# Brochu/RayTrace-WE-GPU

Hardware: AMD Instinct MI355X
Metric: Msamples/sec (pixels x spp) at 1920x1080 spp=100 depth=50 (higher is better)
Workload: dtype f32

## Files before the change

raytrace-we-gpu_amd/csrc/rtx_api.hip:

```cpp
#include <hip/hip_runtime.h>

#include <algorithm>
#include <cmath>
#include <cstdio>
#include <cstring>
#include <new>
#include <string>
#include <vector>

#include "../../include/rtx.h"
#include "rtx_internal.h"
#include "rtx_prefilter.h"

namespace {

thread_local std::string g_last_error;

int fail(int code, const std::string &msg) {
    g_last_error = msg;
    return code;
}

int hip_fail(hipError_t e, const char *what) {
    return fail(RTX_ERR_HIP, std::string(what) + ": " + hipGetErrorString(e));
// ... 724 lines not shown
    if (c->chain_n != 0 && std::memcmp(f, &c->chain_frame, sizeof *f) != 0) c->chain_n = 0;
    c->frame = *f;
    c->have_frame = true;
    return RTX_OK;
}

uint32_t rtx_part_rows(uint32_t height, uint32_t tile_rows, uint32_t part, uint32_t nparts) {
    if (tile_rows == 0 || nparts == 0 || part >= nparts) return 0;
    const uint32_t tiles = (height + tile_rows - 1) / tile_rows;
    if (part >= tiles) return 0;
    const uint32_t my_tiles = (tiles - part + nparts - 1) / nparts;
    uint32_t rows = my_tiles * tile_rows;
    const uint32_t last_tile = part + (my_tiles - 1) * nparts;
    if (last_tile == tiles - 1) rows -= tiles * tile_rows - height;
    return rows;
}

struct RefineArgs {
    const float4 *chain_in;
    float4 *chain_out;
    uint32_t samples, out_n;
    uint32_t *cost_map;
    uint32_t carry_spp;
};
static size_t chain_bytes(size_t px) { return px * (sizeof(float4) + sizeof(uint32_t)); }
static uint32_t *cost_map_of(const rtx_ctx *c) { return reinterpret_cast<uint32_t *>(c->d_chain + c->chain_pixels); }
static bool cost_map_valid(const rtx_ctx *c) { return c->d_chain && c->chain_n != 0 && c->cost_s_prev != 0; }
static int render_impl(rtx_ctx *c, uint32_t tile_rows, uint32_t part, uint32_t nparts, void *d_out,
                       float4 *accum, uint32_t accum_frames, uint32_t frame_index,
                       const RefineArgs *refine = nullptr);

static size_t sched_state_off(size_t npix) { return (2 * npix + 2 * rtx::kCostBuckets + rtx::kSchedWords + 3) & ~(size_t)3; }
constexpr uint32_t kPromCap = 65536;

int rtx_render_rows(rtx_ctx *c, uint32_t tile_rows, uint32_t part, uint32_t nparts, void *d_out) {
    if (!c) return fail(RTX_ERR_INVALID, "rtx_render_rows: null ctx");
    return render_impl(c, tile_rows, part, nparts, d_out, nullptr, 0, c->frame.frame_index);
}

int rtx_accumulate(rtx_ctx *c, int reset) {
    if (!c) return fail(RTX_ERR_INVALID, "rtx_accumulate: null ctx");
    if (!c->have_frame) return fail(RTX_ERR_STATE, "rtx_accumulate: no frame set");
    int rc = set_device(c);
    if (rc) return rc;
    const size_t px = (size_t)c->frame.width * c->frame.height;
    if (reset || c->accum_frames == 0 || !c->d_accum || c->accum_pixels != px) {
        if (!c->d_accum || c->accum_pixels != px) {
            RTX_HIP(hipStreamSynchronize(c->stream));
            (void)hipFree(c->d_accum);
            c->d_accum = nullptr;
            c->accum_pixels = 0;
            RTX_HIP(hipMalloc(&c->d_accum, px * sizeof(float4)));
            c->accum_pixels = px;
        }
        RTX_HIP(hipMemsetAsync(c->d_accum, 0, px * sizeof(float4), c->stream));
        c->accum_frames = 0;
    }
    rc = render_impl(c, 1, 0, 1, nullptr, c->d_accum, c->accum_frames + 1, c->accum_frames);
    if (rc == RTX_OK) c->accum_frames++;
    return rc;
}

uint32_t rtx_accumulated_frames(rtx_ctx *c) { return c ? c->accum_frames : 0; }

int rtx_render_sum(rtx_ctx *c, uint32_t frame_index, void *d_sum) {
    if (!c) return fail(RTX_ERR_INVALID, "rtx_render_sum: null ctx");
// ... 99 lines not shown
        p.chain_in = refine->chain_in;
        p.chain_out = refine->chain_out;
        p.out_n = refine->out_n;
    }

    if (c->ev_count == c->events.size()) {
        EventPair &old = c->events[c->ev_head];
        const hipError_t q = hipEventQuery(old.stop);
        if (q == hipSuccess) {
            float t = 0.0f;
            RTX_HIP(hipEventElapsedTime(&t, old.start, old.stop));
            c->ms_folded += t;
            c->ev_head = (c->ev_head + 1) % c->events.size();
            c->ev_count--;
        } else if (q == hipErrorNotReady) {
            std::vector<EventPair> grown(2 * c->events.size());
            for (size_t i = 0; i < c->ev_count; ++i) grown[i] = c->events[(c->ev_head + i) % c->events.size()];
            c->events.swap(grown);
            c->ev_head = 0;
        } else {
            return hip_fail(q, "hipEventQuery");
        }
    }
    EventPair &ev = c->events[(c->ev_head + c->ev_count) % c->events.size()];
    if (!ev.start) RTX_HIP(hipEventCreate(&ev.start));
    if (!ev.stop) RTX_HIP(hipEventCreate(&ev.stop));
    RTX_HIP(hipEventRecord(ev.start, c->stream));
    const size_t npix = (size_t)rows * f.width;
    if (c->sched_pixels < npix) {
        RTX_HIP(hipStreamSynchronize(c->stream));
        (void)hipFree(c->d_sched);
        c->d_sched = nullptr;
        c->sched_pixels = 0;
        RTX_HIP(hipMalloc(&c->d_sched,
                          (sched_state_off(npix) + 4 * npix + 8 * (size_t)kPromCap + 5 * npix) * sizeof(uint32_t)));
        RTX_HIP(hipMemsetAsync(c->d_sched + sched_state_off(npix) + 4 * npix, 0,
                               8 * (size_t)kPromCap * sizeof(uint32_t), c->stream));
        c->sched_pixels = npix;
    }
    const size_t ps_need = rtx::ps_scratch_floats(p);
    if (ps_need > c->ps_floats) {
        RTX_HIP(hipStreamSynchronize(c->stream));
        (void)hipFree(c->d_ps);
        c->d_ps = nullptr;
        c->ps_floats = 0;
        RTX_HIP(hipMalloc(&c->d_ps, ps_need * sizeof(float)));
        c->ps_floats = ps_need;
    }
    rtx::KSchedule sched;
    sched.ps_scratch = c->d_ps;
    sched.ps_floats = c->ps_floats;
    sched.cost = c->d_sched;
    sched.perm = c->d_sched + c->sched_pixels;
    sched.buckets = c->d_sched + 2 * c->sched_pixels;
    sched.state = reinterpret_cast<float4 *>(c->d_sched + sched_state_off(c->sched_pixels));
    sched.npix = (uint32_t)c->sched_pixels;
    sched.nbuckets = rtx::kCostBuckets;
    sched.tune = c->tune;
    if (!c->aux_stream) {
        RTX_HIP(hipStreamCreateWithFlags(&c->aux_stream, hipStreamNonBlocking));
        RTX_HIP(hipEventCreateWithFlags(&c->ev_fork, hipEventDisableTiming));
        RTX_HIP(hipEventCreateWithFlags(&c->ev_join, hipEventDisableTiming));
    }
    sched.aux = c->aux_stream;
    sched.prom_q = c->d_sched + sched_state_off(c->sched_pixels) + 4 * c->sched_pixels;
    sched.prom_cap = kPromCap;
    sched.stage = reinterpret_cast<float4 *>(sched.prom_q + 8 * (size_t)kPromCap);
    sched.inv = sched.prom_q + 8 * (size_t)kPromCap + 4 * c->sched_pixels;
    sched.epoch = (uint32_t)++c->epoch;
    sched.ev_fork = c->ev_fork;
    sched.ev_join = c->ev_join;
    sched.cost_map = refine ? refine->cost_map : nullptr;
    sched.carry_spp = refine ? refine->carry_spp : 0u;
    hipError_t e = rtx::launch_render(p, sched, c->stream);
    if (e != hipSuccess) return hip_fail(e, "launch_render");
    RTX_HIP(hipEventRecord(ev.stop, c->stream));
    c->ev_count++;
    c->launches++;
    c->samples += (uint64_t)rows * f.width * p.spp;
    return RTX_OK;
}

int rtx_render(rtx_ctx *c) { return rtx_render_rows(c, 1, 0, 1, nullptr); }

int rtx_refine(rtx_ctx *c, uint32_t samples, int reset) {
    if (!c) return fail(RTX_ERR_INVALID, "rtx_refine: null ctx");
    if (samples == 0) return fail(RTX_ERR_INVALID, "rtx_refine: samples is 0");
    if (!c->have_world) return fail(RTX_ERR_STATE, "rtx_refine: no world uploaded");
    if (!c->have_frame) return fail(RTX_ERR_STATE, "rtx_refine: no frame set");
    if (c->frame.rng_mode == RTX_RNG_PER_SAMPLE)
        return fail(RTX_ERR_INVALID, "rtx_refine: the per-sample RNG has no chain to continue (rtx_accumulate is its "
                                     "progressive form)");
    const size_t px = (size_t)c->frame.width * c->frame.height;
    const bool fresh = reset || c->chain_n == 0 || !c->d_chain || c->chain_pixels != px ||
                       std::memcmp(&c->frame, &c->chain_frame, sizeof c->frame) != 0;
    const uint32_t have = fresh ? 0u : c->chain_n;
    if (samples > 0xffffffffu - have) return fail(RTX_ERR_INVALID, "rtx_refine: more than 2^32 - 1 samples in all");
    int rc = set_device(c);
    if (rc) return rc;
    if (!c->d_chain || c->chain_pixels != px) {
        RTX_HIP(hipStreamSynchronize(c->stream));
// ... 373 lines not shown
```

raytrace-we-gpu_amd/csrc/rtx_diag.h:

```cpp
#pragma once

#include "rtx_internal.h"

#ifndef RTX_DIAG_PROF
#define RTX_DIAG_PROF 0
#endif
#ifndef RTX_DIAG_PIXEL
#define RTX_DIAG_PIXEL 0
#endif
#ifndef RTX_DIAG_COOP
#define RTX_DIAG_COOP 0
#endif
#ifndef RTX_DIAG_RAYS
#define RTX_DIAG_RAYS 0
#endif

namespace rtx {
namespace {

#if RTX_DIAG_PROF
__device__ __forceinline__ uint32_t *diag_slots() {
    __shared__ uint32_t s[4][8];
    return s[(threadIdx.x / 64) & 3u];
}
__device__ __forceinline__ void diag_add(int k, uint32_t v) {
    const uint64_t m = __ballot(1);
    if ((int)(threadIdx.x & 63u) == __ffsll((long long)m) - 1) diag_slots()[k] += v;
}
#define RTX_DIAG_ADD(k, v) diag_add(k, v)
__device__ __forceinline__ unsigned long long *diag_hw() {
    __shared__ unsigned long long s[4][8];
    return s[(threadIdx.x / 64) & 3u];
}
__device__ __forceinline__ void diag_hw_clock(int k) {
    const uint64_t m = __ballot(1);
    if ((int)(threadIdx.x & 63u) == __ffsll((long long)m) - 1) {
        const unsigned long long tn = __builtin_readcyclecounter();
        if (k >= 0) diag_hw()[k] += tn - diag_hw()[3];
        diag_hw()[3] = tn;
    }
}
__device__ __forceinline__ void diag_hw_walk(uint32_t steps, uint32_t rounds) {
    uint32_t mx = 0;
    for (int b = 7; b >= 0; --b) {
        const uint32_t t = mx | (1u << b);
        if (__ballot(min(steps, 255u) >= t) != 0ull) mx = t;
    }
    const uint64_t m = __ballot(1);
    if ((int)(threadIdx.x & 63u) == __ffsll((long long)m) - 1) {
        diag_hw()[4] += 1ull;
        diag_hw()[5] += mx;
        diag_hw()[7] += rounds ? rounds : mx;
    }
    atomicAdd(&diag_hw()[6], (unsigned long long)steps);
}
#define RTX_DIAG_HW_BEGIN() diag_hw_clock(-1)
#define RTX_DIAG_HW(k) diag_hw_clock(k)
#define RTX_DIAG_WALK(steps, rounds) diag_hw_walk(steps, rounds)
#else
#define RTX_DIAG_ADD(k, v)
#define RTX_DIAG_HW_BEGIN()
#define RTX_DIAG_HW(k)
#define RTX_DIAG_WALK(steps, rounds)
#endif

#define RTX_CP(k)                                                   \
    if (RTX_DIAG_COOP && cp) {                                      \
        const unsigned long long tn = __builtin_readcyclecounter(); \
        cp[k] += tn - *tq;                                          \
        *tq = tn;                                                   \
    }

struct Diag {
#if RTX_DIAG_RAYS
    uint32_t rit = 0;
#endif
#if RTX_DIAG_PROF
    unsigned long long pr[7] = {0, 0, 0, 0, 0, 0, 0};
    unsigned long long tq = 0;
#endif
#if RTX_DIAG_COOP
    unsigned long long cpa[8] = {0, 0, 0, 0, 0, 0, 0, 0};
    unsigned long long ctq = 0;
    bool was_coop = false;
#endif
    __device__ __forceinline__ void begin() {
#if RTX_DIAG_PROF
        if ((threadIdx.x & 63u) == 0u)
            for (int k = 0; k < 8; ++k) diag_slots()[k] = 0u, diag_hw()[k] = 0ull;
        tq = __builtin_readcyclecounter();
#endif
#if RTX_DIAG_COOP
        ctq = __builtin_readcyclecounter();
#endif
    }
    __device__ __forceinline__ void section(int k) {
#if RTX_DIAG_PROF
        const unsigned long long tn = __builtin_readcyclecounter();
        pr[k] += tn - tq;
        tq = tn;
#else
        (void)k;
#endif
    }
    __device__ __forceinline__ void iteration(uint64_t act) {
#if RTX_DIAG_PROF
        pr[4]++;
        pr[6] += __popcll(act);
#else
        (void)act;
#endif
    }
    __device__ __forceinline__ void tail_iteration() {
#if RTX_DIAG_PROF
        pr[5]++;
#endif
    }
    __device__ __forceinline__ unsigned long long *coop_begin(uint32_t tier, unsigned long long *&tqp) {
#if RTX_DIAG_COOP
        tqp = &ctq;
        if (tier != (uint32_t)RTX_DIAG_COOP) return nullptr;
        const unsigned long long tn = __builtin_readcyclecounter();
// ... 15 lines not shown
        }
        was_coop = tier == (uint32_t)RTX_DIAG_COOP;
#else
        (void)cp;
        (void)tier;
#endif
    }
    __device__ __forceinline__ void rays(const KParams &P, f3 o, f3 d, bool live, uint32_t slot) {
#if RTX_DIAG_RAYS
        if (!P.wave_times) return;
        const uint32_t w = blockIdx.x * (blockDim.x / 64u) + threadIdx.x / 64u;
        if ((++rit + w * 13u) % (uint32_t)RTX_DIAG_RAYS != 0u) return;
        unsigned long long r = 0;
        if ((threadIdx.x & 63u) == 0u) r = atomicAdd(&P.wave_times[0], 1ull);
        r = __shfl(r, 0, 64);
        const unsigned long long base = 64ull + 256ull * r;
        if (base + 256ull > 2ull * P.wave_cap) return;
        auto pk = [](float a, float b) {
            return ((unsigned long long)__float_as_uint(b) << 32) | __float_as_uint(a);
        };
        unsigned long long *q = P.wave_times + base + 4u * (threadIdx.x & 63u);
        q[0] = pk(o.x, o.y);
        q[1] = pk(o.z, d.x);
        q[2] = pk(d.y, d.z);
        q[3] = ((unsigned long long)slot << 32) | (live ? 1u : 0u);
#else
        (void)P, (void)o, (void)d, (void)live, (void)slot;
#endif
    }
    __device__ __forceinline__ void finish(const KParams &P) {
#if RTX_DIAG_PROF
        if (P.wave_times && (threadIdx.x & 63u) == 0u) {
            for (int k = 0; k < 7; ++k) atomicAdd(&P.wave_times[k], pr[k]);
            for (int k = 0; k < 7; ++k) atomicAdd(&P.wave_times[8 + k], (unsigned long long)diag_slots()[k]);
            if (P.wave_cap >= 12u)
                for (int k = 0; k < 8; ++k) atomicAdd(&P.wave_times[16 + k], diag_hw()[k]);
        }
#endif
#if RTX_DIAG_COOP
        if (P.wave_times && (threadIdx.x & 63u) == 0u)
            for (int k = 0; k < 6; ++k) atomicAdd(&P.wave_times[k], cpa[k]);
#endif
        (void)P;
    }
};

__device__ __forceinline__ void diag_pixel_start(const KParams &P, uint32_t gid, unsigned long long mode) {
#if RTX_DIAG_PIXEL
    if (P.wave_times && gid < P.wave_cap) P.wave_times[2 * gid] = (__builtin_amdgcn_s_memrealtime() << 2) | mode;
#else
    (void)P;
    (void)gid;
    (void)mode;
#endif
}
__device__ __forceinline__ void diag_pixel_end(const KParams &P, uint32_t gid) {
#if RTX_DIAG_PIXEL
    if (P.wave_times && gid < P.wave_cap) P.wave_times[2 * gid + 1] = __builtin_amdgcn_s_memrealtime();
#else
    (void)P;
    (void)gid;
#endif
}
constexpr bool kDiagAny = RTX_DIAG_PROF || RTX_DIAG_PIXEL || RTX_DIAG_COOP || RTX_DIAG_RAYS;

}
}
```

raytrace-we-gpu_amd/csrc/rtx_internal.h:

```cpp
#pragma once

#include <hip/hip_runtime.h>
#include <stdint.h>

#include "rtx_grid.h"
#include "rtx_refine_keys.h"

struct rtx_ctx;

namespace rtx {

struct KScene {
    const float *soa;
    const float *pre;
    const float4 *pre4;
    const float4 *cen;
    const int *mtype;
    const float4 *mval;
    uint32_t n, n_pad;
    float smag;
    float flat_cy;
    uint32_t flat_lo, flat_hi;
    const float *cpre;
    const float *cbnd;
// ... 62 lines not shown
    float4 *accum;
    uint32_t accum_frames;
    unsigned long long *wave_times;
    uint32_t wave_cap;
    const uint32_t *perm;
    uint32_t *cost_out;
    uint32_t cost_spp;
    uint32_t cost_cap;
    uint32_t cost_capped;
    uint32_t *pre_done;
    uint32_t pre_stop;
    float4 *state;
    uint32_t prio_slots;
    uint32_t coop_max;
    uint32_t prio_t1, prio_t2, prio_hot;
    uint32_t trace_ext;
    uint32_t chunk;
    uint32_t *prom;
    uint32_t *errors;
    unsigned long long *err_diag;
    uint32_t *prom_q;
    uint32_t prom_cap, prom_min, epoch;
    uint32_t *heavy;
    const uint32_t *cost_in;
    float dyn_bar[3];
    uint32_t trace_lg;
    float *ps_scratch;
    uint32_t ps_px, ps_cap;
    const float4 *chain_in;
    float4 *chain_out;
    uint32_t out_n;
    uint32_t *cost_map;
    uint32_t carry_spp;
};

struct KTune {
    double a1, a1_small, a1_low, a2_small, a2_medium, a2_large, rho, rho_low, rho2, prio_frac;
    double occ_small, occ_low, occ_normal;
    uint32_t coop_max;
    uint32_t coop_max_large;
    uint32_t prio_t1, prio_t2, prio_hot;
    uint32_t chunk;
    double trace_small, trace_low, trace_medium, trace_large;
    double prom_small, prom_low, prom_medium, prom_large;
    double prom_big;
    uint32_t trace_group;
    double trace_solo;
    uint32_t cap_split;
    double dyn1, dyn2, dyn3;
};
KTune default_tune();

struct KSchedule {
    uint32_t *cost;
    uint32_t *perm;
    float4 *state;
    float4 *stage;
    uint32_t *inv;
    uint32_t *buckets;
    uint32_t npix;
    uint32_t nbuckets;
    float *ps_scratch;
    size_t ps_floats;
    KTune tune;
    hipStream_t aux;
    hipEvent_t ev_fork, ev_join;
    uint32_t *prom_q;
    uint32_t prom_cap;
    uint32_t epoch;
    uint32_t *cost_map;
    uint32_t carry_spp;
};
constexpr uint32_t kSchedWords = 16;
constexpr uint32_t kBlock = 256;

hipError_t launch_render(const KParams &p, const KSchedule &sched, hipStream_t stream);
size_t ps_scratch_floats(const KParams &p);
hipError_t launch_cost(const KParams &p, hipStream_t stream);
hipError_t launch_deinterleave(const float4 *gathered, float4 *image, uint32_t width,
                               uint32_t height, uint32_t tile_rows, uint32_t nparts,
                               uint32_t max_rows, hipStream_t stream);
hipError_t launch_fold_frames(float4 *accum, const float4 *sums, uint32_t m, size_t slot_pixels, size_t pixels,
                              uint32_t divisor, float4 *image, hipStream_t stream);
hipError_t launch_chain_image(const float4 *chain, float4 *image, size_t pixels, uint32_t n, hipStream_t stream);
hipError_t launch_debug_hit_world(const KScene &s, const float *rays, uint32_t nrays,
                                  float t_min, float t_max, uint32_t start_block, float *out,
                                  hipStream_t stream);
bool debug_scan_rate_supported(const KParams &p);
hipError_t launch_debug_scan_rate(const KParams &p, uint32_t reps, unsigned long long *sink, uint32_t *waves,
                                  hipStream_t stream);
hipError_t launch_debug_math(int fn, const float *in0, const float *in1, uint32_t n,
// ... 8 lines not shown
```

raytrace-we-gpu_amd/csrc/rtx_kernels.hip:

```cpp
#include <algorithm>
#include <cstdlib>
#include <cstring>
#include <mutex>
#include <type_traits>
#include <vector>

#include "rtx_device_math.h"
#include "rtx_diag.h"
#include "rtx_internal.h"
#include "rtx_prefilter.h"

#if defined(__HIP_DEVICE_COMPILE__) && !defined(__gfx950__)
#error "rtx_kernels.hip targets gfx950 (MI355X) only"
#endif

namespace rtx {

namespace {

constexpr float kTMin = 0.001f;

struct FrameVals {
    f3 org, hor, ver, llc;
    float img_w, img_h;
// ... 1472 lines not shown
    return true;
}

template <bool kCost = false, bool kRefine = false>
__device__ __forceinline__ bool shade(const KParams &P, const Frame &F, Lane &L, int hit, float t,
                                      uint32_t prom_thr = 0u) {
    L.segs++;
    f3 c;
    const int r = path_segment(P, L, hit, t, c);
    if (r == kSegSky) L.acc = L.acc + c;
    const bool ended = r != kSegContinue;
    if (ended) {
        L.sample++;
        if (L.sample >= P.spp) {
            write_pixel<kCost, kRefine>(P, L);
            L.active = false;
            diag_pixel_end(P, L.gid);
        } else if (!kCost && prom_thr != 0u && promote<kRefine>(P, L, prom_thr)) {
            L.active = false;
            return true;
        } else {
            begin_sample(P, F, L.x, L.y, L);
        }
    } else if (kCost && P.cost_cap != 0u && L.segs - L.seg0 >= P.cost_cap) {
        P.cost_out[L.gid] = P.cost_capped;
        P.state[L.gid] = make_float4(0.0f, 0.0f, 0.0f, __uint_as_float(0x7fc00000u));
        L.segs = L.seg0;
        L.active = false;
        diag_pixel_end(P, L.gid);
    }
    return false;
}

__device__ __forceinline__ void lane_pixel(const KParams &P, uint32_t gid, uint32_t &x, uint32_t &y) {
    const uint32_t lr = gid / P.width;
    x = gid - lr * P.width;
    const uint32_t j = lr / P.tile_rows;
    const uint32_t w = lr - j * P.tile_rows;
    y = (j * P.nparts + P.part) * P.tile_rows + w;
}

__device__ __forceinline__ void count_segments(const KParams &P, uint32_t segs) {
#pragma unroll
    for (int off = 32; off > 0; off >>= 1) segs += __shfl_xor(segs, off, 64);
    if ((threadIdx.x & 63u) == 0u && segs != 0u) atomicAdd(P.counters, (unsigned long long)segs);
}

#ifndef RTX_CHECK_KERNARG
#define RTX_CHECK_KERNARG 0
#endif
__device__ __forceinline__ Frame load_frame(const KParams &P) {
    if constexpr (RTX_CHECK_KERNARG != 0) {
        const FrameVals v = frame_vals();
        const bool same = __float_as_uint(v.img_w) == __float_as_uint(P.img_w) &&
                          __float_as_uint(v.img_h) == __float_as_uint(P.img_h) &&
                          __float_as_uint(v.org.x) == __float_as_uint(P.org[0]) &&
                          __float_as_uint(v.llc.z) == __float_as_uint(P.llc[2]) &&
                          __float_as_uint(v.lens_r) == __float_as_uint(P.lens_r);
        if (!same && P.errors && (threadIdx.x & 63u) == 0u) atomicOr(P.errors, kErrKernarg);
    }
    return Frame{};
}

template <bool kRefine = false>
__device__ __forceinline__ void start_pixel(const KParams &P, const Frame &F, uint32_t gid, Lane &L) {
    L.gid = gid;
    lane_pixel(P, gid, L.x, L.y);
    L.seg0 = L.segs;
    const float4 st = P.state && !P.cost_out ? P.state[gid] : make_float4(0.f, 0.f, 0.f, 0.f);
    L.c0 = 0u;
    if (P.state && !P.cost_out && !__builtin_isnan(st.w)) {
        L.acc = mk3(st.x, st.y, st.z);
        L.sample = P.cost_spp;
        L.seed = st.w;
        if constexpr (kRefine) {
            L.c0 = P.cost_map[gid];
        } else if (P.cost_in) {
            L.c0 = P.cost_in[gid];
        }
    } else {
        L.acc = mk3(0.0f, 0.0f, 0.0f);
        L.sample = 0;
        L.seed = pixel_seed(P, L.x, L.y, 0);
        if constexpr (kRefine) {
            if (P.chain_in) {
                const float4 ch = P.chain_in[gid];
                L.acc = mk3(ch.x, ch.y, ch.z);
                L.seed = ch.w;
            }
            if (P.carry_spp != 0u) L.c0 = P.cost_map[gid];
        }
        if (P.state && !P.cost_out) L.seg0 |= kSeg0Restart;
    }
    L.active = true;
    begin_sample(P, F, L.x, L.y, L);
}

__device__ __forceinline__ void set_prio(uint32_t p) {
    switch (__builtin_amdgcn_readfirstlane(p)) {
        case 0: __builtin_amdgcn_s_setprio(0); break;
        case 1: __builtin_amdgcn_s_setprio(1); break;
        case 2: __builtin_amdgcn_s_setprio(2); break;
        default: __builtin_amdgcn_s_setprio(3); break;
    }
}

template <bool kRefine = false>
__device__ __forceinline__ uint32_t dyn_level(const KParams &P, const Lane &L, float m) {
    float rem = 0.0f;
    if (L.active) {
        const bool rs = (L.seg0 & kSeg0Restart) != 0u;
        const float segs = (float)(L.segs - (L.seg0 & ~kSeg0Restart) + L.c0);
        rem = rs && L.sample == 0u ? 3.0e38f : segs * (float)(P.spp - L.sample) / (float)max(L.sample, 1u);
        if constexpr (kRefine) {
            const float all = (float)(L.segs - (L.seg0 & ~kSeg0Restart)) + (float)L.c0;
            rem = rs && L.sample == 0u ? 3.0e38f
                                       : all * (float)(P.spp - L.sample) /
                                             fmaxf((float)L.sample + (float)P.carry_spp, 1.0f);
        }
    }
    return __ballot(rem > P.dyn_bar[2] * m) != 0ull   ? 3u
           : __ballot(rem > P.dyn_bar[1] * m) != 0ull ? 2u
           : __ballot(rem > P.dyn_bar[0] * m) != 0ull ? 1u
                                                      : 0u;
}

template <bool kRefine = false>
__device__ __forceinline__ bool refill(const KParams &P, const Frame &F, uint32_t lo, uint32_t hi, Lane &L) {
    const uint64_t idle = __ballot(!L.active);
    if (idle == 0ull) return false;
    const uint32_t cnt = (uint32_t)__popcll(idle);
    if (P.chunk > 1u) {
        const uint32_t lane = threadIdx.x & 63u;
        const uint32_t rank = (uint32_t)__popcll(idle & ((1ull << lane) - 1ull));
        const uint32_t avail = L.ce - L.cb;
        uint32_t nb = 0, n = 0;
        if (cnt > avail) {
            n = cnt - avail;
            if (L.cb < hi - (hi - lo) / 8u) n = max(n, P.chunk);
            if (lane == 0u) nb = atomicAdd(P.queue, n);
            nb = lo + (uint32_t)__shfl((int)nb, 0, 64);
        }
        if (!L.active) {
            const uint32_t g = rank < avail ? L.cb + rank : nb + (rank - avail);
            if (g < hi) {
                start_pixel<kRefine>(P, F, P.perm ? P.perm[g] : g, L);
                L.slot = g;
                diag_pixel_start(P, L.gid, 0);
            }
        }
        if (cnt > avail) {
            L.cb = nb + (cnt - avail);
            L.ce = min(nb + n, hi);
            return L.cb >= hi;
        }
        L.cb += cnt;
        return false;
    }
    const int leader = __ffsll((long long)idle) - 1;
    const uint32_t lane = threadIdx.x & 63u;
    uint32_t base = 0;
    if ((int)lane == leader) base = atomicAdd(P.queue, cnt);
    base = lo + __shfl(base, leader, 64);
    if (!L.active) {
        const uint32_t g = base + (uint32_t)__popcll(idle & ((1ull << lane) - 1ull));
        if (g < hi) {
            start_pixel<kRefine>(P, F, P.perm ? P.perm[g] : g, L);
            L.slot = g;
            diag_pixel_start(P, L.gid, 0);
        }
    }
    return base + cnt >= hi;
}

struct HeavyState {
    uint32_t k1, kh;
    bool t1_done, t2_done;
    uint32_t tier;
};
template <bool kRefine = false>
__device__ __forceinline__ bool take_from(const KParams &P, const Frame &F, uint32_t *ctr, uint32_t lo, uint32_t hi,
                                          uint32_t room, uint64_t act, Lane &L, bool &done) {
    const uint32_t lane = threadIdx.x & 63u;
    uint32_t h = 0;
    if (lane == 0u) h = atomicAdd(ctr, room);
    h = lo + __shfl(h, 0, 64);
    if (h >= hi) {
        done = true;
        return false;
    }
    const uint32_t take = min(room, hi - h);
    const uint32_t rk = (uint32_t)__popcll(~act & ((1ull << lane) - 1ull));
    if (!L.active && rk < take) {
        start_pixel<kRefine>(P, F, P.perm[h + rk], L);
        L.slot = h + rk;
        diag_pixel_start(P, L.gid, ctr == P.heavy ? 1ull : 2ull);
    }
    if (h + room >= hi) done = true;
    return true;
}
template <bool kRefine = false>
__device__ __forceinline__ void take_heavy(const KParams &P, const Frame &F, HeavyState &H, Lane &L) {
    const uint64_t act = __ballot(L.active);
    const uint32_t have = (uint32_t)__popcll(act);
    if (have == 0u) H.tier = 0;
    if (have == 0u && !H.t1_done && take_from<kRefine>(P, F, P.heavy, 0, H.k1, kHeavy1, act, L, H.t1_done)) {
        H.tier = 1;
        return;
    }
    if (H.tier == 1u) return;
    if (!H.t2_done && have < kHeavy2 && take_from<kRefine>(P, F, P.heavy + 2, H.k1, H.kh, kHeavy2 - have, act, L, H.t2_done))
        H.tier = 2;
}

template <uint32_t kLg, typename Src>
__device__ __forceinline__ void trace_group_segment(const KParams &P, const Frame &F, const Src &src, Lane &W,
                                                    bool &ended) {
    constexpr uint32_t lg = kLg;
    const KScene &S = P.scene;
    const uint32_t lane = threadIdx.x & 63u;
    const uint32_t g = 1u << lg, k = lane & (g - 1u);
    const uint64_t gm = lg >= 6u ? ~0ull : ((1ull << g) - 1ull) << (lane & ~(g - 1u));
    const float inf = __uint_as_float(0x7f800000u);
    const int last = (int)S.n - 1;
    const ScatterSpec sp = scatter_spec(W.seed);
    LineTest T = line_test_setup(W.o.x, W.o.y, W.o.z, W.d.x, W.d.y, W.d.z, W.a, S.smag);
    if (lg < 6u && !W.active) {
        T.ux = T.uy = T.uz = T.vy = T.vz = T.nou = T.nov = 0.0f;
        T.thr = inf;
    }
    const f2v ux = {T.ux, T.ux}, uy = {T.uy, T.uy}, uz = {T.uz, T.uz}, vy = {T.vy, T.vy}, vz = {T.vz, T.vz};
    const f2v nou = {T.nou, T.nou}, nov = {T.nov, T.nov}, th = {T.thr, T.thr};
    uint64_t key = hit_key(inf, -1);
    bool ok = true;
    const uint32_t nsteps = src.npairs >> lg;
#pragma unroll 1
    for (uint32_t s0 = 0; s0 < nsteps; s0 += kGfSteps) {
        uint32_t im = 0;
        const uint32_t s1 = min(s0 + kGfSteps, nsteps);
        auto step = [&](uint32_t st) {
            f2v cx, cy, cz, R;
            src.pair((st << lg) + k, cx, cy, cz, R);
            const f2v pu = fma2(cx, ux, fma2(cy, uy, fma2(cz, uz, nou)));
            const f2v pv = fma2(cy, vy, fma2(cz, vz, nov));
// ... 264 lines not shown
    if (kPF && threadIdx.x == 0) *pack = 0u;
    if (prom_on && threadIdx.x == 0) s_server = 0u;
    if (prom_on && blockIdx.x == 0 && threadIdx.x == 0)
        __hip_atomic_store(&P.prom[3], 1u, __ATOMIC_RELAXED, __HIP_MEMORY_SCOPE_AGENT);
    if (coop_lds || kPF || prom_on) __syncthreads();
    const int last = (int)P.scene.n - 1;
    const Frame F = load_frame(P);
    const uint32_t npix = P.rows_local * P.width;
    const unsigned long long t_start = P.wave_times ? __builtin_amdgcn_s_memrealtime() : 0ull;
    Lane L;
    L.active = false;
    L.segs = 0;
    L.slot = ~0u;
    L.cb = L.ce = 0u;
    bool exhausted = !kPersist;
    if (!kPersist) {
        const uint32_t gid = tile_pixel(blockIdx.x * kRB + threadIdx.x, P.width, P.rows_local, kExactTile);
        if (gid < npix) start_pixel<kRefine>(P, F, gid, L);
    }
    HeavyState H;
    H.kh = (kPersist && P.heavy) ? min(P.heavy[1], npix) : 0u;
    H.k1 = (kPersist && P.heavy) ? min(P.heavy[3], H.kh) : 0u;
    H.t1_done = H.k1 == 0u || P.trace_ext != 0u;
    H.t2_done = H.k1 == H.kh;
    H.tier = 0;
    const uint32_t kh = H.kh;
    const float dyn_m = (kPersist && P.cost_in && P.heavy) ? __uint_as_float(P.heavy[5]) : 0.0f;
    const uint32_t owned = npix - (P.trace_ext != 0u ? H.k1 : 0u);
    uint32_t written = 0;
    unsigned long long last_beat = 0;
    Diag D;
    D.begin();
    for (;;) {
        if (!(H.t1_done && H.t2_done) && (H.tier != 0u || __ballot(L.active) == 0ull)) take_heavy<kRefine>(P, F, H, L);
        if (H.tier != 0u && __ballot(L.active) == 0ull) H.tier = 0;
        const bool heavy = H.tier != 0u;
        if (!heavy && !exhausted) exhausted = refill<kRefine>(P, F, kh, npix, L);
        if (kPersist && kCost && P.pre_done && exhausted && pre_stop(P, npix, L)) continue;
        const uint64_t act = __ballot(L.active);
        D.section(0);
        if (act == 0ull) {
            if (!prom_on) break;
            if (written != 0u && (threadIdx.x & 63u) == 0u)
                __hip_atomic_fetch_add(&P.prom[2], written, __ATOMIC_RELAXED, __HIP_MEMORY_SCOPE_AGENT);
            written = 0;
            uint32_t srv = 0;
            if ((threadIdx.x & 63u) == 0u) srv = atomicCAS(&s_server, 0u, threadIdx.x / 64u + 1u);
            srv = (uint32_t)__builtin_amdgcn_readfirstlane(__shfl((int)srv, 0, 64));
            if (srv != 0u && srv != threadIdx.x / 64u + 1u) break;
            if (!take_promoted<kRefine>(P, F, npix, owned, false, L)) {
                if ((threadIdx.x & 63u) == 0u) atomicExch(&s_server, 0u);
                break;
            }
            L.active = (threadIdx.x & 63u) == 0u;
            H.tier = 1;
            continue;
        }
        const uint64_t was_active = act;
        if (prom_on) beat(P, last_beat);
        D.iteration(act);
        if (heavy || (exhausted && (uint32_t)__popcll(act) <= P.coop_max)) {
            D.tail_iteration();
            float my_best = __uint_as_float(0x7f800000u);
            bool my_seq = false;
            set_prio(H.tier == 1u ? P.prio_t1 : H.tier == 2u ? P.prio_t2 : (uint32_t)kTailPrio);
            unsigned long long *ctqp;
            unsigned long long *cp = D.coop_begin(H.tier, ctqp);
            bool promoted = false;
            int my_hit = kCulled
                             ? hit_world_groups_culled(P.scene, act, L.active, L.o, L.d, L.a, L.inv_a, kTMin, coop_ws,
// ... 159 lines not shown
    const uint32_t k1 = min(P.heavy[3], min(P.heavy[1], npix));
    const uint32_t k0 = min(P.heavy[4], k1);
    const uint32_t lane = threadIdx.x & 63u;
    const uint32_t lg_many = min(max(P.trace_lg, 3u), 6u);
    set_prio(P.prio_t1);
    uint32_t lg = 6u;
    Lane W;
    W.active = false;
    W.segs = 0;
    W.seg0 = 0;
    W.slot = 0;
    uint32_t segs = 0;
    bool t1_done = k1 == 0u;
    bool serve_done = P.prom == nullptr;
    unsigned long long last_beat = 0;
    for (;;) {
        uint64_t act = __ballot(W.active);
        if (act == 0ull && t1_done) lg = lg_many;
        if (!t1_done) {
            if (act == 0ull) {
                const uint32_t next = (uint32_t)__builtin_amdgcn_readfirstlane(
                    __hip_atomic_load(P.heavy, __ATOMIC_RELAXED, __HIP_MEMORY_SCOPE_AGENT));
                lg = next < k0 ? 6u : lg_many;
            }
            const uint32_t g = 1u << lg;
            const uint64_t need = __ballot(!W.active && (lane & (g - 1u)) == 0u);
            if (need != 0ull) {
                const uint32_t n = (uint32_t)__popcll(need);
                uint32_t base = 0;
                if (lane == 0u) base = atomicAdd(P.heavy, n);
                base = (uint32_t)__builtin_amdgcn_readfirstlane(__shfl((int)base, 0, 64));
                const uint32_t rank = (uint32_t)__popcll(need & ((1ull << (lane & ~(g - 1u))) - 1ull));
                if (!W.active && base + rank < k1) {
                    start_pixel<kRefine>(P, F, P.perm[base + rank], W);
                    W.slot = base + rank;
                    diag_pixel_start(P, W.gid, 1ull);
                }
                if (base + n >= k1) t1_done = true;
                act = __ballot(W.active);
            }
        }
        if (t1_done && !serve_done) {
            const uint32_t g = 1u << lg;
            const uint64_t need = __ballot(!W.active && (lane & (g - 1u)) == 0u);
            if (need != 0ull) {
                set_prio(P.prio_t1);
                if (take_promoted_groups<kRefine>(P, F, npix, npix - k1, need, lg, act == 0ull, W) < 0) serve_done = true;
                set_prio(P.prio_t1);
                act = __ballot(W.active);
            }
        }
        if (act == 0ull) {
            if (t1_done && serve_done) break;
            continue;
        }
        if (t1_done && lg < 6u) {
            uint32_t m = 0;
            for (uint32_t r = 0; r < (64u >> lg); ++r) m += (uint32_t)((act >> (r << lg)) & 1ull);
            if (2u * m <= (64u >> lg)) {
                const uint32_t nlg = 6u - (m <= 1u ? 0u : 32u - (uint32_t)__builtin_clz(m - 1u));
                regroup(W, lg, nlg, act);
                lg = nlg;
            }
        }
        bool ended;
        const bool first = (lane & ((1u << lg) - 1u)) == 0u;
        if (lg == 6u) {
            uint32_t n = 0;
// ... 53 lines not shown
constexpr uint32_t kChunkShare = 16;

__global__ void __launch_bounds__(kBlock) k_cost_hist(const uint32_t *cost, uint32_t width, uint32_t rows,
                                                      uint32_t cost_spp, uint32_t sat_cap, uint32_t tile,
                                                      uint32_t tile_y, uint32_t *counts) {
    __shared__ uint32_t h[kCostBuckets];
    for (uint32_t b = threadIdx.x; b < kCostBuckets; b += kBlock) h[b] = 0;
    __syncthreads();
    const uint32_t base = blockIdx.x * kBlock * kSortPerThread;
    for (uint32_t k = 0; k < kSortPerThread; ++k) {
        const uint32_t i = tile_pixel(base + k * kBlock + threadIdx.x, width, rows, tile, tile_y);
        if (i != ~0u) atomicAdd(&h[cost_key(cost, i, width, rows, cost_spp, sat_cap)], 1u);
    }
    __syncthreads();
    for (uint32_t b = threadIdx.x; b < kCostBuckets; b += kBlock)
        if (h[b]) atomicAdd(&counts[b], h[b]);
}
__global__ void __launch_bounds__(kBlock) k_carried_hist(const uint32_t *map, uint32_t width, uint32_t rows,
                                                         uint32_t s_prev, uint32_t tile, uint32_t tile_y,
                                                         uint32_t *counts) {
    __shared__ uint32_t h[kCostBuckets];
    for (uint32_t b = threadIdx.x; b < kCostBuckets; b += kBlock) h[b] = 0;
    __syncthreads();
    const uint32_t base = blockIdx.x * kBlock * kSortPerThread;
    for (uint32_t k = 0; k < kSortPerThread; ++k) {
        const uint32_t i = tile_pixel(base + k * kBlock + threadIdx.x, width, rows, tile, tile_y);
        if (i != ~0u) atomicAdd(&h[carried_key(map, i, width, rows, s_prev)], 1u);
    }
    __syncthreads();
    for (uint32_t b = threadIdx.x; b < kCostBuckets; b += kBlock)
        if (h[b]) atomicAdd(&counts[b], h[b]);
}

__global__ void __launch_bounds__(kBlock) k_cost_scatter(const uint32_t *cost, uint32_t width, uint32_t rows,
                                                         uint32_t cost_spp, uint32_t sat_cap, uint32_t tile,
                                                         uint32_t tile_y,
                                                         const uint32_t *counts, uint32_t *cursors,
                                                         uint32_t *perm, uint32_t *inv) {
    __shared__ uint32_t h[kCostBuckets], start[kCostBuckets];
    for (uint32_t b = threadIdx.x; b < kCostBuckets; b += kBlock) h[b] = 0;
    __syncthreads();
    const uint32_t base = blockIdx.x * kBlock * kSortPerThread;
    uint32_t rank[kSortPerThread], key[kSortPerThread];
    for (uint32_t k = 0; k < kSortPerThread; ++k) {
        const uint32_t i = tile_pixel(base + k * kBlock + threadIdx.x, width, rows, tile, tile_y);
        key[k] = i != ~0u ? cost_key(cost, i, width, rows, cost_spp, sat_cap) : 0u;
        rank[k] = i != ~0u ? atomicAdd(&h[key[k]], 1u) : 0u;
    }
    __syncthreads();
    if (threadIdx.x == 0) {
        uint32_t pre = 0;
        for (uint32_t b = 0; b < kCostBuckets; ++b) {
            start[b] = pre;
            pre += counts[b];
        }
    }
    __syncthreads();
    for (uint32_t b = threadIdx.x; b < kCostBuckets; b += kBlock)
        if (h[b]) start[b] += atomicAdd(&cursors[b], h[b]);
    __syncthreads();
    for (uint32_t k = 0; k < kSortPerThread; ++k) {
        const uint32_t i = tile_pixel(base + k * kBlock + threadIdx.x, width, rows, tile, tile_y);
        if (i != ~0u) {
            const uint32_t g = start[key[k]] + rank[k];
            perm[g] = i;
            if (inv) inv[i] = g;
        }
    }
}
__global__ void __launch_bounds__(kBlock) k_carried_scatter(const uint32_t *map, uint32_t width, uint32_t rows,
                                                            uint32_t s_prev, uint32_t tile, uint32_t tile_y,
                                                            const uint32_t *counts, uint32_t *cursors,
                                                            uint32_t *perm, uint32_t *inv) {
    __shared__ uint32_t h[kCostBuckets], start[kCostBuckets];
    for (uint32_t b = threadIdx.x; b < kCostBuckets; b += kBlock) h[b] = 0;
    __syncthreads();
    const uint32_t base = blockIdx.x * kBlock * kSortPerThread;
    uint32_t rank[kSortPerThread], key[kSortPerThread];
    for (uint32_t k = 0; k < kSortPerThread; ++k) {
        const uint32_t i = tile_pixel(base + k * kBlock + threadIdx.x, width, rows, tile, tile_y);
        key[k] = i != ~0u ? carried_key(map, i, width, rows, s_prev) : 0u;
        rank[k] = i != ~0u ? atomicAdd(&h[key[k]], 1u) : 0u;
    }
    __syncthreads();
    if (threadIdx.x == 0) {
        uint32_t pre = 0;
        for (uint32_t b = 0; b < kCostBuckets; ++b) {
            start[b] = pre;
            pre += counts[b];
        }
    }
    __syncthreads();
    for (uint32_t b = threadIdx.x; b < kCostBuckets; b += kBlock)
        if (h[b]) start[b] += atomicAdd(&cursors[b], h[b]);
    __syncthreads();
    for (uint32_t k = 0; k < kSortPerThread; ++k) {
        const uint32_t i = tile_pixel(base + k * kBlock + threadIdx.x, width, rows, tile, tile_y);
        if (i != ~0u) {
            const uint32_t g = start[key[k]] + rank[k];
            perm[g] = i;
            if (inv) inv[i] = g;
        }
    }
}

}
KTune default_tune() {
    KTune t;
    t.a1 = kHeavy1Alpha;
    t.a1_small = kHeavy1AlphaSmall;
    t.a1_low = kHeavy1AlphaLow;
    t.a2_small = kHeavyAlpha;
    t.a2_medium = kHeavy2AlphaMedium;
    t.a2_large = kHeavy2AlphaLarge;
    t.rho = kHeavyRho;
    t.rho_low = kHeavyRhoLow;
    t.rho2 = kHeavyRho2;
    t.prio_frac = kPrioFracX100 / 100.0;
    t.occ_small = t.occ_low = t.occ_normal = 1.0;
    t.coop_max = (uint32_t)kCoopMax;
    t.coop_max_large = (uint32_t)kCoopMaxLarge;
    t.prio_t1 = 3;
    t.prio_t2 = 2;
    t.prio_hot = 3;
    t.chunk = 64;
    t.trace_small = kTraceSmall;
    t.trace_low = kTraceLow;
    t.trace_medium = kTraceMedium;
    t.trace_large = kTraceLarge;
    t.prom_small = kPromSmall;
    t.prom_low = kPromLow;
    t.prom_medium = kPromMedium;
    t.prom_large = kPromLarge;
    t.prom_big = kPromBig;
// ... 615 lines not shown
            c.pre_stop = (uint32_t)(kPreStopFrac * (double)pblocks * kRB);
        }
        launch_kr<true, true>(p.scene, pblocks, lds, stream, c);
    } else {
        launch_kr<false, true>(p.scene, need_x, lds, stream, c);
    }
#ifndef RTX_QUEUE_TILE_ALL
#define RTX_QUEUE_TILE_ALL 0
#endif
#ifndef RTX_QUEUE_TILE_SPLIT
#define RTX_QUEUE_TILE_SPLIT 0
#endif
    uint32_t qtile = RTX_QUEUE_TILE_ALL || (double)lanes >= tune.rho * (double)min(need, resident_blocks(render_fn<true, false>(p.scene), lds)) * kRB
                         ? kQueueTile
                         : 0u;
    uint32_t qtile_y = 0u;
    if (RTX_QUEUE_TILE_SPLIT != 0 && p.nparts > 1u && p.tile_rows != 0u) qtile = RTX_QUEUE_TILE_SPLIT, qtile_y = p.tile_rows;
    const uint32_t sblocks = ceil_div(tile_span(p.width, p.rows_local, qtile, qtile_y), kBlock * kSortPerThread);
    if (carried)
        hipLaunchKernelGGL(k_carried_hist, dim3(sblocks), dim3(kBlock), 0, stream, sched.cost_map, p.width,
                           p.rows_local, sched.carry_spp, qtile, qtile_y, sched.buckets);
    else
        hipLaunchKernelGGL(k_cost_hist, dim3(sblocks), dim3(kBlock), 0, stream, sched.cost, p.width,
                           p.rows_local, c.spp, split_cap, qtile, qtile_y, sched.buckets);
    uint32_t blocks = min(need, resident_blocks(render_fn<true, false>(p.scene), lds));
    {
        const double px_per_lane = (double)lanes / ((double)blocks * kRB);
        const double occ = px_per_lane < tune.rho ? tune.occ_small : px_per_lane < tune.rho_low ? tune.occ_low : tune.occ_normal;
        blocks = max(1u, (uint32_t)(blocks * occ + 0.5));
    }
    uint32_t *heavy = sched.buckets + 2 * kCostBuckets;
    hipLaunchKernelGGL(k_heavy_split, dim3(1), dim3(64), 0, stream, sched.buckets, (uint32_t)lanes, blocks * kRB, p.spp,
                       heavy, tune);
    if (carried)
        hipLaunchKernelGGL(k_carried_scatter, dim3(sblocks), dim3(kBlock), 0, stream, sched.cost_map, p.width,
                           p.rows_local, sched.carry_spp, qtile, qtile_y, sched.buckets, sched.buckets + kCostBuckets,
                           sched.perm, sched.stage ? sched.inv : nullptr);
    else
        hipLaunchKernelGGL(k_cost_scatter, dim3(sblocks), dim3(kBlock), 0, stream, sched.cost, p.width,
                           p.rows_local, c.spp, split_cap, qtile, qtile_y, sched.buckets, sched.buckets + kCostBuckets, sched.perm,
                           sched.stage ? sched.inv : nullptr);
    KParams q = p;
    q.cost_spp = carried ? 0u : c.spp;
    q.perm = sched.perm;
    q.out_slot = sched.stage;
    q.stage_tag = sched.epoch;
    q.state = carried ? nullptr : sched.state;
    q.carry_spp = carried ? sched.carry_spp : 0u;
    q.prio_slots = (uint32_t)((double)blocks * kRB * tune.prio_frac);
    q.heavy = heavy;
    if (tune.dyn1 > 0.0) {
        q.cost_in = carried ? sched.cost_map : sched.cost;
        q.dyn_bar[0] = (float)tune.dyn1;
        q.dyn_bar[1] = (float)tune.dyn2;
        q.dyn_bar[2] = (float)tune.dyn3;
    }
    {
        const double ppl = (double)lanes / ((double)blocks * kRB);
        q.chunk = (!pf && ppl >= tune.rho2) ? min(tune.chunk, 4096u)
                  : ppl >= tune.rho_low     ? min(tune.chunk, kChunkShare)
                                            : 0u;
    }
    e = hipMemsetAsync(p.queue, 0, sizeof(uint32_t), stream);
    if (e != hipSuccess) return e;
    uint32_t trace_waves = 0;
    if (sched.aux && !pf && p.scene.n <= kCoopLds) {
        const double px_per_lane = (double)lanes / ((double)blocks * kRB);
        const double frac = px_per_lane < tune.rho ? tune.trace_small : px_per_lane < tune.rho_low ? tune.trace_low
                            : px_per_lane < tune.rho2 ? tune.trace_medium : tune.trace_large;
        trace_waves = (uint32_t)(frac * blocks * (kRB / 64) + 0.5);
    }
    {
        const double px_per_lane = (double)lanes / ((double)blocks * kRB);
        const double pm = p.scene.n > kCoopLds    ? tune.prom_big
                          : px_per_lane < tune.rho ? tune.prom_small : px_per_lane < tune.rho_low ? tune.prom_low
                          : px_per_lane < tune.rho2 ? tune.prom_medium : tune.prom_large;
        if (pm > 0.0 && sched.prom_q && sched.prom_cap > 0) {
// ... 105 lines not shown
```

Baseline: 6477.

## Precompute packed per-slot start records in scatter kernel to cut dependent loads

The cost/carried scatter kernels now also write a 32-byte start record per sorted slot, holding pixel index, coordinates, c0 cost and resume state. The render kernel's refill and heavy-take paths then load one contiguous record instead of chasing perm[g] and then gathering state[gid], cost_in[gid] and recomputing pixel coordinates. This is meant to replace a dependent chain of scattered loads at pixel start with coalesced sequential loads. In exchange it adds extra global writes in the scatter pass and 8 words per pixel of scratch memory. Optional diagnostic counters for load latency are added as well.

Result: no change. 6516, median of 6 (+0.6%).

```diff
diff --git a/raytrace-we-gpu_amd/csrc/rtx_api.hip b/raytrace-we-gpu_amd/csrc/rtx_api.hip
--- a/raytrace-we-gpu_amd/csrc/rtx_api.hip
+++ b/raytrace-we-gpu_amd/csrc/rtx_api.hip
@@ -780,6 +780,9 @@
 
 static size_t sched_state_off(size_t npix) { return (2 * npix + 2 * rtx::kCostBuckets + rtx::kSchedWords + 3) & ~(size_t)3; }
 constexpr uint32_t kPromCap = 65536;
+static size_t sched_rec_off(size_t npix) {
+    return (sched_state_off(npix) + 4 * npix + 8 * (size_t)kPromCap + 5 * npix + 7) & ~(size_t)7;
+}
 
 int rtx_render_rows(rtx_ctx *c, uint32_t tile_rows, uint32_t part, uint32_t nparts, void *d_out) {
     if (!c) return fail(RTX_ERR_INVALID, "rtx_render_rows: null ctx");
@@ -945,8 +948,7 @@
         (void)hipFree(c->d_sched);
         c->d_sched = nullptr;
         c->sched_pixels = 0;
-        RTX_HIP(hipMalloc(&c->d_sched,
-                          (sched_state_off(npix) + 4 * npix + 8 * (size_t)kPromCap + 5 * npix) * sizeof(uint32_t)));
+        RTX_HIP(hipMalloc(&c->d_sched, (sched_rec_off(npix) + 8 * npix) * sizeof(uint32_t)));
         RTX_HIP(hipMemsetAsync(c->d_sched + sched_state_off(npix) + 4 * npix, 0,
                                8 * (size_t)kPromCap * sizeof(uint32_t), c->stream));
         c->sched_pixels = npix;
@@ -980,6 +982,7 @@
     sched.prom_cap = kPromCap;
     sched.stage = reinterpret_cast<float4 *>(sched.prom_q + 8 * (size_t)kPromCap);
     sched.inv = sched.prom_q + 8 * (size_t)kPromCap + 4 * c->sched_pixels;
+    sched.rec = reinterpret_cast<uint4 *>(c->d_sched + sched_rec_off(c->sched_pixels));
     sched.epoch = (uint32_t)++c->epoch;
     sched.ev_fork = c->ev_fork;
     sched.ev_join = c->ev_join;
diff --git a/raytrace-we-gpu_amd/csrc/rtx_diag.h b/raytrace-we-gpu_amd/csrc/rtx_diag.h
--- a/raytrace-we-gpu_amd/csrc/rtx_diag.h
+++ b/raytrace-we-gpu_amd/csrc/rtx_diag.h
@@ -20,7 +20,7 @@
 
 #if RTX_DIAG_PROF
 __device__ __forceinline__ uint32_t *diag_slots() {
-    __shared__ uint32_t s[4][8];
+    __shared__ uint32_t s[4][16];
     return s[(threadIdx.x / 64) & 3u];
 }
 __device__ __forceinline__ void diag_add(int k, uint32_t v) {
@@ -28,6 +28,16 @@
     if ((int)(threadIdx.x & 63u) == __ffsll((long long)m) - 1) diag_slots()[k] += v;
 }
 #define RTX_DIAG_ADD(k, v) diag_add(k, v)
+#if RTX_DIAG_PROF >= 2
+__device__ __forceinline__ unsigned long long diag_loads_begin() { return __builtin_readcyclecounter(); }
+__device__ __forceinline__ void diag_loads_end(unsigned long long t0) {
+    asm volatile("s_waitcnt vmcnt(0)" ::: "memory");
+    diag_add(7, (uint32_t)(__builtin_readcyclecounter() - t0));
+}
+#define RTX_DIAG_LOADS_BEGIN() const unsigned long long diag_ld0 = diag_loads_begin()
+#define RTX_DIAG_LOADS_END() diag_loads_end(diag_ld0)
+#define RTX_DIAG_START_END() (diag_add(8, (uint32_t)(__builtin_readcyclecounter() - diag_ld0)), diag_add(9, 1u))
+#endif
 __device__ __forceinline__ unsigned long long *diag_hw() {
     __shared__ unsigned long long s[4][8];
     return s[(threadIdx.x / 64) & 3u];
@@ -63,6 +73,11 @@
 #define RTX_DIAG_HW(k)
 #define RTX_DIAG_WALK(steps, rounds)
 #endif
+#ifndef RTX_DIAG_LOADS_BEGIN
+#define RTX_DIAG_LOADS_BEGIN() ((void)0)
+#define RTX_DIAG_LOADS_END() ((void)0)
+#define RTX_DIAG_START_END() ((void)0)
+#endif
 
 #define RTX_CP(k)                                                   \
     if (RTX_DIAG_COOP && cp) {                                      \
@@ -87,7 +102,7 @@
     __device__ __forceinline__ void begin() {
 #if RTX_DIAG_PROF
         if ((threadIdx.x & 63u) == 0u)
-            for (int k = 0; k < 8; ++k) diag_slots()[k] = 0u, diag_hw()[k] = 0ull;
+            for (int k = 0; k < 8; ++k) diag_slots()[k] = diag_slots()[8 + k] = 0u, diag_hw()[k] = 0ull;
         tq = __builtin_readcyclecounter();
 #endif
 #if RTX_DIAG_COOP
@@ -169,9 +184,11 @@
 #if RTX_DIAG_PROF
         if (P.wave_times && (threadIdx.x & 63u) == 0u) {
             for (int k = 0; k < 7; ++k) atomicAdd(&P.wave_times[k], pr[k]);
-            for (int k = 0; k < 7; ++k) atomicAdd(&P.wave_times[8 + k], (unsigned long long)diag_slots()[k]);
+            for (int k = 0; k < 8; ++k) atomicAdd(&P.wave_times[8 + k], (unsigned long long)diag_slots()[k]);
             if (P.wave_cap >= 12u)
                 for (int k = 0; k < 8; ++k) atomicAdd(&P.wave_times[16 + k], diag_hw()[k]);
+            if (P.wave_cap >= 16u)
+                for (int k = 0; k < 8; ++k) atomicAdd(&P.wave_times[24 + k], (unsigned long long)diag_slots()[8 + k]);
         }
 #endif
 #if RTX_DIAG_COOP
diff --git a/raytrace-we-gpu_amd/csrc/rtx_internal.h b/raytrace-we-gpu_amd/csrc/rtx_internal.h
--- a/raytrace-we-gpu_amd/csrc/rtx_internal.h
+++ b/raytrace-we-gpu_amd/csrc/rtx_internal.h
@@ -118,6 +118,18 @@
     uint32_t out_n;
     uint32_t *cost_map;
     uint32_t carry_spp;
+    const uint4 *rec;
+};
+
+constexpr uint32_t kRecResume = 0u;
+constexpr uint32_t kRecRestart = 1u;
+constexpr uint32_t kRecFresh = 2u;
+constexpr uint32_t kRecKindShift = 30u;
+struct KRecArgs {
+    uint4 *rec;
+    const float4 *state;
+    const uint32_t *c0;
+    uint32_t tile_rows, part, nparts;
 };
 
 struct KTune {
@@ -143,6 +155,7 @@
     float4 *state;
     float4 *stage;
     uint32_t *inv;
+    uint4 *rec;
     uint32_t *buckets;
     uint32_t npix;
     uint32_t nbuckets;
diff --git a/raytrace-we-gpu_amd/csrc/rtx_kernels.hip b/raytrace-we-gpu_amd/csrc/rtx_kernels.hip
--- a/raytrace-we-gpu_amd/csrc/rtx_kernels.hip
+++ b/raytrace-we-gpu_amd/csrc/rtx_kernels.hip
@@ -1528,12 +1528,16 @@
     return false;
 }
 
+__device__ __forceinline__ void part_pixel(uint32_t width, uint32_t tile_rows, uint32_t part, uint32_t nparts,
+                                           uint32_t gid, uint32_t &x, uint32_t &y) {
+    const uint32_t lr = gid / width;
+    x = gid - lr * width;
+    const uint32_t j = lr / tile_rows;
+    const uint32_t w = lr - j * tile_rows;
+    y = (j * nparts + part) * tile_rows + w;
+}
 __device__ __forceinline__ void lane_pixel(const KParams &P, uint32_t gid, uint32_t &x, uint32_t &y) {
-    const uint32_t lr = gid / P.width;
-    x = gid - lr * P.width;
-    const uint32_t j = lr / P.tile_rows;
-    const uint32_t w = lr - j * P.tile_rows;
-    y = (j * P.nparts + P.part) * P.tile_rows + w;
+    part_pixel(P.width, P.tile_rows, P.part, P.nparts, gid, x, y);
 }
 
 __device__ __forceinline__ void count_segments(const KParams &P, uint32_t segs) {
@@ -1558,11 +1562,17 @@
     return Frame{};
 }
 
-template <bool kRefine = false>
+#ifndef RTX_START_REC
+#define RTX_START_REC 1
+#endif
+constexpr bool kStartRec = RTX_START_REC != 0;
+
+template <bool kRefine = false, bool kProfLoads = false>
 __device__ __forceinline__ void start_pixel(const KParams &P, const Frame &F, uint32_t gid, Lane &L) {
     L.gid = gid;
     lane_pixel(P, gid, L.x, L.y);
     L.seg0 = L.segs;
+    RTX_DIAG_LOADS_BEGIN();
     const float4 st = P.state && !P.cost_out ? P.state[gid] : make_float4(0.f, 0.f, 0.f, 0.f);
     L.c0 = 0u;
     if (P.state && !P.cost_out && !__builtin_isnan(st.w)) {
@@ -1574,6 +1584,7 @@
         } else if (P.cost_in) {
             L.c0 = P.cost_in[gid];
         }
+        if constexpr (kProfLoads) RTX_DIAG_LOADS_END();
     } else {
         L.acc = mk3(0.0f, 0.0f, 0.0f);
         L.sample = 0;
@@ -1586,10 +1597,53 @@
             }
             if (P.carry_spp != 0u) L.c0 = P.cost_map[gid];
         }
+        if constexpr (kProfLoads) RTX_DIAG_LOADS_END();
         if (P.state && !P.cost_out) L.seg0 |= kSeg0Restart;
     }
     L.active = true;
     begin_sample(P, F, L.x, L.y, L);
+}
+
+template <bool kRefine = false, bool kProfLoads = false, bool kRec = kStartRec>
+__device__ __forceinline__ void start_slot(const KParams &P, const Frame &F, uint32_t g, Lane &L) {
+    L.slot = g;
+    if constexpr (!kRec) {
+        RTX_DIAG_LOADS_BEGIN();
+        const uint32_t gid = P.perm ? P.perm[g] : g;
+        if constexpr (kProfLoads) RTX_DIAG_LOADS_END();
+        start_pixel<kRefine, kProfLoads>(P, F, gid, L);
+        return;
+    }
+    RTX_DIAG_LOADS_BEGIN();
+    const uint4 *r = P.rec + 2u * (size_t)g;
+    const uint4 a = r[0], b = r[1];
+    if constexpr (kProfLoads) RTX_DIAG_LOADS_END();
+    const uint32_t kind = b.w >> kRecKindShift;
+    L.gid = b.x;
+    L.c0 = b.y;
+    L.x = b.z;
+    L.y = b.w & ((1u << kRecKindShift) - 1u);
+    L.seg0 = L.segs;
+    if (kind == kRecResume) {
+        L.acc = mk3(__uint_as_float(a.x), __uint_as_float(a.y), __uint_as_float(a.z));
+        L.sample = P.cost_spp;
+        L.seed = __uint_as_float(a.w);
+    } else {
+        L.acc = mk3(0.0f, 0.0f, 0.0f);
+        L.sample = 0;
+        L.seed = pixel_seed(P, L.x, L.y, 0);
+        if constexpr (kRefine) {
+            if (P.chain_in) {
+                const float4 ch = P.chain_in[L.gid];
+                L.acc = mk3(ch.x, ch.y, ch.z);
+                L.seed = ch.w;
+            }
+        }
+        if (kind == kRecRestart) L.seg0 |= kSeg0Restart;
+    }
+    L.active = true;
+    begin_sample(P, F, L.x, L.y, L);
+    if constexpr (kProfLoads) RTX_DIAG_START_END();
 }
 
 __device__ __forceinline__ void set_prio(uint32_t p) {
@@ -1621,7 +1675,7 @@
                                                       : 0u;
 }
 
-template <bool kRefine = false>
+template <bool kRefine = false, bool kRec = kStartRec>
 __device__ __forceinline__ bool refill(const KParams &P, const Frame &F, uint32_t lo, uint32_t hi, Lane &L) {
     const uint64_t idle = __ballot(!L.active);
     if (idle == 0ull) return false;
@@ -1640,8 +1694,7 @@
         if (!L.active) {
             const uint32_t g = rank < avail ? L.cb + rank : nb + (rank - avail);
             if (g < hi) {
-                start_pixel<kRefine>(P, F, P.perm ? P.perm[g] : g, L);
-                L.slot = g;
+                start_slot<kRefine, true, kRec>(P, F, g, L);
                 diag_pixel_start(P, L.gid, 0);
             }
         }
@@ -1661,8 +1714,7 @@
     if (!L.active) {
         const uint32_t g = base + (uint32_t)__popcll(idle & ((1ull << lane) - 1ull));
         if (g < hi) {
-            start_pixel<kRefine>(P, F, P.perm ? P.perm[g] : g, L);
-            L.slot = g;
+            start_slot<kRefine, true, kRec>(P, F, g, L);
             diag_pixel_start(P, L.gid, 0);
         }
     }
@@ -1674,7 +1726,7 @@
     bool t1_done, t2_done;
     uint32_t tier;
 };
-template <bool kRefine = false>
+template <bool kRefine = false, bool kRec = kStartRec>
 __device__ __forceinline__ bool take_from(const KParams &P, const Frame &F, uint32_t *ctr, uint32_t lo, uint32_t hi,
                                           uint32_t room, uint64_t act, Lane &L, bool &done) {
     const uint32_t lane = threadIdx.x & 63u;
@@ -1688,24 +1740,23 @@
     const uint32_t take = min(room, hi - h);
     const uint32_t rk = (uint32_t)__popcll(~act & ((1ull << lane) - 1ull));
     if (!L.active && rk < take) {
-        start_pixel<kRefine>(P, F, P.perm[h + rk], L);
-        L.slot = h + rk;
+        start_slot<kRefine, false, kRec>(P, F, h + rk, L);
         diag_pixel_start(P, L.gid, ctr == P.heavy ? 1ull : 2ull);
     }
     if (h + room >= hi) done = true;
     return true;
 }
-template <bool kRefine = false>
+template <bool kRefine = false, bool kRec = kStartRec>
 __device__ __forceinline__ void take_heavy(const KParams &P, const Frame &F, HeavyState &H, Lane &L) {
     const uint64_t act = __ballot(L.active);
     const uint32_t have = (uint32_t)__popcll(act);
     if (have == 0u) H.tier = 0;
-    if (have == 0u && !H.t1_done && take_from<kRefine>(P, F, P.heavy, 0, H.k1, kHeavy1, act, L, H.t1_done)) {
+    if (have == 0u && !H.t1_done && take_from<kRefine, kRec>(P, F, P.heavy, 0, H.k1, kHeavy1, act, L, H.t1_done)) {
         H.tier = 1;
         return;
     }
     if (H.tier == 1u) return;
-    if (!H.t2_done && have < kHeavy2 && take_from<kRefine>(P, F, P.heavy + 2, H.k1, H.kh, kHeavy2 - have, act, L, H.t2_done))
+    if (!H.t2_done && have < kHeavy2 && take_from<kRefine, kRec>(P, F, P.heavy + 2, H.k1, H.kh, kHeavy2 - have, act, L, H.t2_done))
         H.tier = 2;
 }
 
@@ -2036,10 +2087,10 @@
     Diag D;
     D.begin();
     for (;;) {
-        if (!(H.t1_done && H.t2_done) && (H.tier != 0u || __ballot(L.active) == 0ull)) take_heavy<kRefine>(P, F, H, L);
+        if (!(H.t1_done && H.t2_done) && (H.tier != 0u || __ballot(L.active) == 0ull)) take_heavy<kRefine, kStartRec && !kCost>(P, F, H, L);
         if (H.tier != 0u && __ballot(L.active) == 0ull) H.tier = 0;
         const bool heavy = H.tier != 0u;
-        if (!heavy && !exhausted) exhausted = refill<kRefine>(P, F, kh, npix, L);
+        if (!heavy && !exhausted) exhausted = refill<kRefine, kStartRec && !kCost>(P, F, kh, npix, L);
         if (kPersist && kCost && P.pre_done && exhausted && pre_stop(P, npix, L)) continue;
         const uint64_t act = __ballot(L.active);
         D.section(0);
@@ -2265,8 +2316,7 @@
                 base = (uint32_t)__builtin_amdgcn_readfirstlane(__shfl((int)base, 0, 64));
                 const uint32_t rank = (uint32_t)__popcll(need & ((1ull << (lane & ~(g - 1u))) - 1ull));
                 if (!W.active && base + rank < k1) {
-                    start_pixel<kRefine>(P, F, P.perm[base + rank], W);
-                    W.slot = base + rank;
+                    start_slot<kRefine>(P, F, base + rank, W);
                     diag_pixel_start(P, W.gid, 1ull);
                 }
                 if (base + n >= k1) t1_done = true;
@@ -2386,11 +2436,29 @@
         if (h[b]) atomicAdd(&counts[b], h[b]);
 }
 
+__device__ __forceinline__ void write_start_rec(const KRecArgs &A, uint32_t width, uint32_t g, uint32_t i) {
+    uint32_t kind = kRecFresh;
+    uint4 a = make_uint4(0u, 0u, 0u, 0u);
+    if (A.state) {
+        const float4 st = A.state[i];
+        kind = __builtin_isnan(st.w) ? kRecRestart : kRecResume;
+        if (kind == kRecResume)
+            a = make_uint4(__float_as_uint(st.x), __float_as_uint(st.y), __float_as_uint(st.z), __float_as_uint(st.w));
+    }
+    uint4 b;
+    b.x = i;
+    b.y = (kind != kRecRestart && A.c0) ? A.c0[i] : 0u;
+    part_pixel(width, A.tile_rows, A.part, A.nparts, i, b.z, b.w);
+    b.w |= kind << kRecKindShift;
+    A.rec[2u * (size_t)g] = a;
+    A.rec[2u * (size_t)g + 1u] = b;
+}
+
 __global__ void __launch_bounds__(kBlock) k_cost_scatter(const uint32_t *cost, uint32_t width, uint32_t rows,
                                                          uint32_t cost_spp, uint32_t sat_cap, uint32_t tile,
                                                          uint32_t tile_y,
                                                          const uint32_t *counts, uint32_t *cursors,
-                                                         uint32_t *perm, uint32_t *inv) {
+                                                         uint32_t *perm, uint32_t *inv, const KRecArgs R) {
     __shared__ uint32_t h[kCostBuckets], start[kCostBuckets];
     for (uint32_t b = threadIdx.x; b < kCostBuckets; b += kBlock) h[b] = 0;
     __syncthreads();
@@ -2419,13 +2487,14 @@
             const uint32_t g = start[key[k]] + rank[k];
             perm[g] = i;
             if (inv) inv[i] = g;
+            if (R.rec) write_start_rec(R, width, g, i);
         }
     }
 }
 __global__ void __launch_bounds__(kBlock) k_carried_scatter(const uint32_t *map, uint32_t width, uint32_t rows,
                                                             uint32_t s_prev, uint32_t tile, uint32_t tile_y,
                                                             const uint32_t *counts, uint32_t *cursors,
-                                                            uint32_t *perm, uint32_t *inv) {
+                                                            uint32_t *perm, uint32_t *inv, const KRecArgs R) {
     __shared__ uint32_t h[kCostBuckets], start[kCostBuckets];
     for (uint32_t b = threadIdx.x; b < kCostBuckets; b += kBlock) h[b] = 0;
     __syncthreads();
@@ -2454,6 +2523,7 @@
             const uint32_t g = start[key[k]] + rank[k];
             perm[g] = i;
             if (inv) inv[i] = g;
+            if (R.rec) write_start_rec(R, width, g, i);
         }
     }
 }
@@ -3135,17 +3205,25 @@
     uint32_t *heavy = sched.buckets + 2 * kCostBuckets;
     hipLaunchKernelGGL(k_heavy_split, dim3(1), dim3(64), 0, stream, sched.buckets, (uint32_t)lanes, blocks * kRB, p.spp,
                        heavy, tune);
+    KRecArgs ra;
+    ra.rec = kStartRec ? sched.rec : nullptr;
+    ra.state = carried ? nullptr : sched.state;
+    ra.c0 = p.chain_out ? sched.cost_map : tune.dyn1 > 0.0 ? sched.cost : nullptr;
+    ra.tile_rows = p.tile_rows;
+    ra.part = p.part;
+    ra.nparts = p.nparts;
     if (carried)
         hipLaunchKernelGGL(k_carried_scatter, dim3(sblocks), dim3(kBlock), 0, stream, sched.cost_map, p.width,
                            p.rows_local, sched.carry_spp, qtile, qtile_y, sched.buckets, sched.buckets + kCostBuckets,
-                           sched.perm, sched.stage ? sched.inv : nullptr);
+                           sched.perm, sched.stage ? sched.inv : nullptr, ra);
     else
         hipLaunchKernelGGL(k_cost_scatter, dim3(sblocks), dim3(kBlock), 0, stream, sched.cost, p.width,
                            p.rows_local, c.spp, split_cap, qtile, qtile_y, sched.buckets, sched.buckets + kCostBuckets, sched.perm,
-                           sched.stage ? sched.inv : nullptr);
+                           sched.stage ? sched.inv : nullptr, ra);
     KParams q = p;
     q.cost_spp = carried ? 0u : c.spp;
     q.perm = sched.perm;
+    q.rec = ra.rec;
     q.out_slot = sched.stage;
     q.stage_tag = sched.epoch;
     q.state = carried ? nullptr : sched.state;
```
